# jgdumas/plinopt

Measured on AMD Instinct MI355X. Metric: candidate SLPs/sec, higher is better.
Workload: dtype u32

## Files before the change

plinopt_amd/csrc/plo_capi.hip:

```cpp
#include "plo_cse_wave.hip"
#include "plo_cse_batch.hip"
#include "plo_kmethod.hip"
#include "plo_kmethod_batch.hip"
#include "plo_cse_big.hip"
#include "plo_cob.hip"
#include "plo_tril.hip"
#include "plo_lin.hip"
#include "plo_orbit.hip"
#include "plo_orbit_cse.hip"
#include "plo_orbit_growth.hip"
#include "plo_dep.hip"
#include "plo_brent.hip"
#include "../../include/plinopt_hip.h"

#include <algorithm>
#include <atomic>
#include <thread>
#include <chrono>
#include <cstdio>
#include <cstring>
#include <dlfcn.h>
#include <functional>
#include <array>
#include <map>
// ... 560 lines not shown
        for (size_t k = 0; k < rv.size(); ++k) iv[k] = (uint16_t)(std::lower_bound(rv.begin(), rv.end(), inv_mod(rv[k], p)) - rv.begin());
        if ((rc = upload(pl, rv, &B.rval)) || (rc = upload(pl, rt, &B.rtid)) || (rc = upload(pl, iv, &B.invid))) return rc;
        B.nr = (uint32_t)rv.size(); B.mode = 2u;
    }
    B.invtab = nullptr;
    if (p <= (1u << 20)) {
        std::vector<uint32_t> it(p, 0); it[1] = 1;
        for (uint32_t i = 2; i < p; ++i) it[i] = (uint32_t)((uint64_t)(p - p / i) * it[p % i] % p);
        if ((rc = upload(pl, it, &B.invtab))) return rc;
    }
    layout_big_workspace(B, K.wide.has_value());
    if ((rc = size_big_lds(pl, K))) return rc;
    HIPCHK(hipFuncSetAttribute(big_kernel_fn(B), hipFuncAttributeMaxDynamicSharedMemorySize, (int)pl->big_lds));
    if (!pl->d_err) HIPCHK(hipMalloc((void **)&pl->d_err, sizeof(uint32_t)));
    if (!pl->d_best) HIPCHK(hipMalloc((void **)&pl->d_best, sizeof(unsigned long long)));
    if (!pl->d_next) HIPCHK(hipMalloc((void **)&pl->d_next, sizeof(unsigned long long)));
    if (!pl->d_stats) HIPCHK(hipMalloc((void **)&pl->d_stats, plo::BS_COUNT * sizeof(uint32_t)));
    B.selcap = PLO_BIG_SELCAP;
    if (K.selcap) B.selcap = (uint32_t)std::min<long>(PLO_BIG_SELCAP, std::max<long>(1, *K.selcap));
    pl->big = true; pl->waves_per_wg = PLO_BIG_THREADS / 64; pl->lds_bytes = pl->big_lds + (uint32_t)sizeof(plo::BigShared);
    return PLO_OK;
}

int rebuild_big_plan(plo_plan *pl)
{
    for (void *d : pl->big_bufs) (void)hipFree(d);
    pl->big_bufs.clear();
    if (pl->d_ws) { (void)hipFree(pl->d_ws); pl->d_ws = nullptr; pl->ws_slices = 0; }
    return build_big_plan(pl);
}

void print_big_stats(const plo_plan *pl)
{
    using namespace plo;
    uint32_t hs[BS_COUNT] = {0};
    if (hipMemcpy(hs, pl->d_stats, sizeof hs, hipMemcpyDeviceToHost) != hipSuccess) return;
    const uint32_t ncand = hs[BS_SUM_CANDIDATES], *mg = hs + BS_LAST_MERGE_US, *ms = hs + BS_LAST_MERGE_SUM_US, *ph = hs + BS_LAST_PHASE_US, *pg = hs + BS_LAST_PGEN_PHASE_US;
    if (pl->B.defer && ncand) fprintf(stderr, "# big kernel, deferred updates: per candidate %.1f merges (%.2f forced by log/hot pressure), %.0f log records, %.0f hot-table updates; last candidate, merge us: hot->log %u, partition pass %u, sum + write back %u, window %u\n",
            (double)hs[BS_SUM_FULLSCANS] / ncand, (double)hs[BS_SUM_FORCED_MERGES] / ncand, ((double)hs[BS_SUM_LOG_HI] * 4294967296.0 + hs[BS_SUM_LOG_LO]) / ncand, (double)hs[BS_SUM_HOTOPS] / ncand, mg[0], mg[1], mg[2], mg[3]);
    if (pl->B.defer && hs[BS_LAST_MERGE_GROUPS]) fprintf(stderr, "#   merge, sum + write back of the last candidate: %u groups; us: sum (loads + table) %u, scan + write back %u, clear + bounds %u\n", hs[BS_LAST_MERGE_GROUPS], ms[0], ms[1], ms[3]);
    fprintf(stderr, "# big kernel (last candidate): steps %u, full scans %u, level rebuilds %u; phase us: level %u select %u rows %u sweep1 %u flush1 %u sweep2 %u flush2 %u tail %u\n",
            hs[BS_LAST_STEPS], hs[BS_LAST_FULLSCANS], hs[BS_LAST_REBUILDS], ph[0], ph[1], ph[2], ph[3], ph[4], ph[5], ph[6], ph[7]);
    fprintf(stderr, "# big kernel (last candidate): image load + CSE phase %u us, ProgramGen %u us\n", hs[BS_LAST_CSE_US], hs[BS_LAST_PGEN_US]);
    fprintf(stderr, "# big kernel (last candidate): image load alone %u us; ProgramGen us: table fill + flags %u, expand + A1 %u, A2 %u, A3 + B + count %u, Triangle set-up %u, Triangle %u, D %u\n",
            hs[BS_LAST_LOAD_US], pg[0], pg[1], pg[2], pg[3], pg[4], pg[5], pg[6]);
#ifdef PLO_BIG_PROFILE
    { unsigned long long g2[40] = {0}; if (hipMemcpyFromSymbol(g2, HIP_SYMBOL(plo::g_prof2), sizeof g2) == hipSuccess && g2[32]) {
        static const char *cls[4] = {">=256", "64..255", "16..63", "<16"};
        for (int c_ = 0; c_ < 4; ++c_) { fprintf(stderr, "#   rows/step %-8s ms per candidate: level %.1f select %.1f rows %.1f sweep %.1f flush1 %.1f flush2 %.1f tail %.1f\n", cls[c_],
            g2[c_ * 8 + 0] / 1e5 / g2[32], g2[c_ * 8 + 1] / 1e5 / g2[32], g2[c_ * 8 + 2] / 1e5 / g2[32], g2[c_ * 8 + 3] / 1e5 / g2[32], g2[c_ * 8 + 4] / 1e5 / g2[32], (g2[c_ * 8 + 6] + g2[c_ * 8 + 5]) / 1e5 / g2[32], g2[c_ * 8 + 7] / 1e5 / g2[32]); } } }
    { unsigned long long gp[16] = {0};
      if (hipMemcpyFromSymbol(gp, HIP_SYMBOL(plo::g_prof), sizeof gp) != hipSuccess) memset(gp, 0, sizeof gp);
      if (gp[3]) fprintf(stderr, "#   sweep of the steps with >= 256 rows, all candidates: %llu trips by %llu wave-sweeps; cycles per trip: chunk wait + stores %.0f, aggregation of both chunks %.0f, rest of the loop %.0f; per wave-sweep %.0f cycles, %.1f trips; probe rounds per trip %.2f, active lanes per trip %.1f\n", gp[3], gp[5], (double)gp[0] / gp[3], (double)gp[1] / gp[3], (double)gp[2] / gp[3], (double)gp[4] / gp[5], (double)gp[3] / gp[5], (double)gp[6] / gp[3], (double)gp[7] / gp[3]);
      if (gp[3] && pl->B.defer && pl->B.mode == 2u) fprintf(stderr, "#   aggregation of a trip (lane 0 of every wave, big steps), cycles: ratio-id lookup %.0f, pair read %.0f, compare-and-swap %.0f, bitmap + count %.0f\n", (double)gp[14] / gp[3], (double)gp[8] / gp[3], (double)gp[9] / gp[3], (double)gp[10] / gp[3]);
      if ((gp[14] || gp[15]) && !pl->B.defer) fprintf(stderr, "#   flush 1, all candidates: entries whose pair with a has a as SECOND column %llu, with b %llu\n", gp[14], gp[15]);
      if (gp[11]) fprintf(stderr, "#   flush 1 of the steps with >= 256 rows: %llu wave-trips by %llu wave-flushes; cycles per trip: fetch + decode %.0f, probe loads %.0f, stores + bookkeeping %.0f; per wave-flush %.0f cycles, %.1f trips\n", gp[11], gp[13], (double)gp[8] / gp[11], (double)gp[9] / gp[11], (double)gp[10] / gp[11], (double)gp[12] / gp[13], (double)gp[11] / gp[13]);
    }
    { const uint32_t *s1 = hs + BS_PROF_SWEEP1_US, *s2 = hs + BS_PROF_SWEEP2_US, *nb = hs + BS_PROF_STEPS;
      fprintf(stderr, "#   steps by rows/step [>=256, 64.., 16.., <16]: %u %u %u %u; sweep1 us %u %u %u %u; sweep2 us %u %u %u %u; fallbacks %u %u; flushed keys %u %u\n",
            nb[0], nb[1], nb[2], nb[3], s1[0], s1[1], s1[2], s1[3], s2[0], s2[1], s2[2], s2[3], hs[BS_PROF_FALLBACK1], hs[BS_PROF_FALLBACK2], hs[BS_PROF_FLUSHED1], hs[BS_PROF_FLUSHED2]); }
#endif
}

int launch_big(plo_plan *pl, plo::BigJob J, plo_stats_t *st)
{
    const BigLaunchKnobs K;
    uint64_t per_cu = 2;
    if (K.wg_per_cu) per_cu = std::max<uint64_t>(1, (uint64_t)*K.wg_per_cu);
    uint64_t want = std::min<uint64_t>(J.ncand, (uint64_t)g_cus * per_cu);
    if (K.slices) want = std::min<uint64_t>(want, (uint64_t)*K.slices);
    if (want == 0) want = 1;
    if (pl->ws_slices < want) {
        if (pl->d_ws) { (void)hipFree(pl->d_ws); pl->d_ws = nullptr; pl->ws_slices = 0; }
        size_t fr = 0, tot = 0; HIPCHK(hipMemGetInfo(&fr, &tot));
        uint64_t fit = (uint64_t)(fr * 0.85) / pl->B.ws_stride;
        if (fit == 0) return fail(PLO_E_CAPACITY, "not enough HBM for one candidate workspace");
        want = std::min(want, fit);
        HIPCHK(hipMalloc(&pl->d_ws, want * pl->B.ws_stride));
        pl->ws_slices = want;
    }
    const uint64_t grid = std::min<uint64_t>(pl->ws_slices, want);
    pl->B.ws = (uint8_t *)pl->d_ws;
    HIPCHK(hipMemsetAsync(pl->d_next, 0, sizeof(unsigned long long), g_stream));
    HIPCHK(hipMemsetAsync(pl->d_stats, 0, plo::BS_COUNT * sizeof(uint32_t), g_stream));
    J.err = pl->d_err; J.next = pl->d_next; J.stats = pl->d_stats;
    void *args[] = {&pl->B, &J};
    const int err = checked_launch(pl->d_err, st, LaunchShape{grid, pl->lds_bytes, pl->waves_per_wg, pl->algo_bytes},
                                   [&] { (void)hipLaunchKernel(big_kernel_fn(pl->B), dim3((uint32_t)grid), dim3(PLO_BIG_THREADS), args, pl->big_lds, g_stream); });
    if (err < 0) return err;
    if (K.stats) print_big_stats(pl);
    if (err == plo::BERR_TABLE && !pl->B.defer && pl->big_cap_scale < 256u) {
        pl->big_cap_scale *= 4u; ++pl->big_refits;
        const int rc = rebuild_big_plan(pl);
        return rc != PLO_OK ? rc : launch_big(pl, J, st);
    }
    if (err == plo::BERR_TABLE && pl->B.defer && !pl->big_no_defer) {
        pl->big_no_defer = true; ++pl->big_refits;
        const int rc = rebuild_big_plan(pl);
        return rc != PLO_OK ? rc : launch_big(pl, J, st);
    }
    if (err) {
        static const char *names[] = {"pair table", "frequency/row-count mismatch", "column bound", "level list", "window list", "multiplier list", "tie selection", "ProgramGen"};
        uint32_t site = 0; (void)hipMemcpy(&site, pl->d_stats + plo::BS_ERR_SITE, sizeof site, hipMemcpyDeviceToHost);
        return fail(err == plo::BERR_COLS || err == plo::BERR_DM || err == plo::BERR_HL ? PLO_E_CAPACITY : err == plo::BERR_PGEN ? PLO_E_UNSUPPORTED : PLO_E_INTERNAL,
                    std::string("device (HBM variant): ") + (err >= 11 && err <= 18 ? names[err - 11] : "unknown") + " error " + std::to_string(err) + (site ? " (site " + std::to_string(site) + ")" : ""));
    }
    return PLO_OK;
// ... 2456 lines not shown
```

plinopt_amd/csrc/plo_cse_big.hip:

```cpp
#include <hip/hip_runtime.h>
#include <stdint.h>
#include <type_traits>

namespace plo {

#ifndef PLO_BIG_THREADS
#define PLO_BIG_THREADS 512
#endif
#define PLO_BIG_SELCAP 512u
#define PLO_GVB 16u
#define PLO_GVMASK 0xFFFFull
#define PLO_GEMPTY 0xFFFFFFFFFFFF0000ull

struct BigPlan {
    uint32_t m, n, nnz, p, NCmax, hbits, rb, bb, unit, maxf0, M0, multcap, dmcap, hlcap, scr_stride, aggbits, mers, agg_cb, agg_dual, selcap, prune;
    uint64_t mu;
    uint32_t nv, vt_lds;
    uint32_t mode, nr;
    const uint16_t *rtid, *invid;
    const uint32_t *rval;
    const uint32_t *rs, *ent0, *tptr, *trows, *ucount0, *hist0;
    const uint2 *vt;
    const uint32_t *invtab;
    const uint64_t *tab0;
// ... 272 lines not shown
            continue;
        }
        s = (s + 2u) & mask; pr += 2u;
    }
    const unsigned long long cm = __builtin_amdgcn_ballot_w64(claimed != 0xFFFFFFFFu);
    if (cm) {
        const uint32_t lane = threadIdx.x & 63u, leader = (uint32_t)__builtin_ctzll(cm);
        uint32_t base = 0;
        if (lane == leader) base = wg_add(aggn, (uint32_t)__builtin_popcountll(cm));
        base = (uint32_t)__builtin_amdgcn_readlane((int)base, (int)leader);
        if (claimed != 0xFFFFFFFFu) {
            const uint32_t idx = base + (uint32_t)__builtin_popcountll(cm & ((1ull << lane) - 1ull));
            if (idx < listcap) agglist[idx] = (uint16_t)claimed;
        }
    }
    return done;
}

#define PLO_RIDB 10u
#define PLO_RSTRIDE 32u
struct BigTabs { const uint2 *vts; const uint16_t *rtid; const uint32_t *rval; const uint16_t *invid; uint16_t *list; uint32_t *bloom; };
__device__ __forceinline__ bool agg_add_rid(uint32_t *aggk, uint32_t *aggc32, uint32_t aggbits, uint32_t key, uint32_t *aggn, uint16_t *agglist, uint32_t listcap) {
    const uint32_t mask = (1u << aggbits) - 1u;
    uint32_t s = (key * 0x9E3779B1u) >> (32u - aggbits);
    uint32_t claimed = 0xFFFFFFFFu; bool done = false;
    for (uint32_t pr = 0; pr < PLO_AGG_PROBES;) {
        const uint32_t s1 = (s + 1u) & mask;
        const uint32_t k0 = __hip_atomic_load(&aggk[s], __ATOMIC_RELAXED, __HIP_MEMORY_SCOPE_WORKGROUP), k1 = __hip_atomic_load(&aggk[s1], __ATOMIC_RELAXED, __HIP_MEMORY_SCOPE_WORKGROUP);
        const bool hit0 = k0 == key, emp0 = k0 == 0xFFFFFFFFu, first = hit0 || emp0;
        const bool hit = hit0 || (!emp0 && k1 == key), emp = emp0 || (!hit && k1 == 0xFFFFFFFFu);
        const uint32_t t = first ? s : s1;
        if (hit) { wg_add(&aggc32[t >> 1], 1u << ((t & 1u) << 4)); done = true; break; }
        if (emp) {
            const uint32_t old = wg_cas(&aggk[t], 0xFFFFFFFFu, key);
            if (old == 0xFFFFFFFFu || old == key) { if (old != key) claimed = t; wg_add(&aggc32[t >> 1], 1u << ((t & 1u) << 4)); done = true; break; }
            continue;
        }
        s = (s + 2u) & mask; pr += 2u;
    }
    const unsigned long long cm = __builtin_amdgcn_ballot_w64(claimed != 0xFFFFFFFFu);
    if (cm) {
        const uint32_t lane = threadIdx.x & 63u, leader = (uint32_t)__builtin_ctzll(cm);
        uint32_t base = 0;
        if (lane == leader) base = wg_add(aggn, (uint32_t)__builtin_popcountll(cm));
        base = (uint32_t)__builtin_amdgcn_readlane((int)base, (int)leader);
        if (claimed != 0xFFFFFFFFu) {
            const uint32_t idx = base + (uint32_t)__builtin_popcountll(cm & ((1ull << lane) - 1ull));
            if (idx < listcap) agglist[idx] = (uint16_t)claimed;
        }
    }
    return done;
}

__device__ __forceinline__ bool agg_add_rid_bm(uint32_t *aggk, uint32_t *aggc32, uint32_t aggbits, uint32_t key, uint32_t *bm, uint32_t hshift, uint32_t *iters = nullptr) {
    const uint32_t pmask = (1u << (aggbits - 1u)) - 1u;
    uint32_t pi = (uint32_t)__umul24(key, 0x9E3779u) >> hshift;
    for (uint32_t left = PLO_AGG_PROBES / 2u;;) {
        if (iters) ++*iters;
        const unsigned long long kk = __hip_atomic_load((unsigned long long *)aggk + pi, __ATOMIC_RELAXED, __HIP_MEMORY_SCOPE_WORKGROUP);
        const uint32_t k0 = (uint32_t)kk, k1 = (uint32_t)(kk >> 32);
        const bool first = k0 == key || k0 == 0xFFFFFFFFu;
        const uint32_t kt = first ? k0 : k1;
        bool mine = kt == key;
        const uint32_t next = !mine && kt != 0xFFFFFFFFu ? 1u : 0u;
        if (kt == 0xFFFFFFFFu) {
            const uint32_t sec = first ? 0u : 1u;
            const uint32_t old = wg_cas((uint32_t *)((unsigned long long *)aggk + pi) + sec, 0xFFFFFFFFu, key);
            if (old == 0xFFFFFFFFu) { const uint32_t t = 2u * pi + sec; wg_or(&bm[t >> 5], 1u << (t & 31u)); }
            mine = old == 0xFFFFFFFFu || old == key;
        }
        if (mine) wg_add(&aggc32[pi], first ? 1u : 0x10000u);
        pi = (pi + next) & pmask; left -= next;
        if (mine || left == 0u) return mine;
    }
}

#ifdef PLO_BIG_PROFILE
__device__ __forceinline__ bool agg_add_rid_first_prof(uint32_t *aggk, uint32_t *aggc32, uint32_t aggbits, uint32_t key, uint32_t *bm, unsigned long long *acc) {
    const unsigned long long c0 = clock64();
    const uint32_t s = ((uint32_t)__umul24(key, 0x9E3779u) >> (32u - aggbits)) & ~1u;
    const unsigned long long kk = __hip_atomic_load((unsigned long long *)(aggk + s), __ATOMIC_RELAXED, __HIP_MEMORY_SCOPE_WORKGROUP);
    const uint32_t k0 = (uint32_t)kk, k1 = (uint32_t)(kk >> 32);
    asm volatile("s_waitcnt lgkmcnt(0)" ::: "memory"); const unsigned long long c1 = clock64();
    const bool hit0 = k0 == key, hit = hit0 || k1 == key, emp0 = k0 == 0xFFFFFFFFu, tryc = !hit && (emp0 || k1 == 0xFFFFFFFFu);
    const uint32_t sec = hit ? (hit0 ? 0u : 1u) : (emp0 ? 0u : 1u), t = s + sec;
    uint32_t old = 0u;
    if (tryc) old = wg_cas(&aggk[t], 0xFFFFFFFFu, key);
    asm volatile("s_waitcnt lgkmcnt(0)" ::: "memory"); const unsigned long long c2 = clock64();
    const bool fresh = tryc && old == 0xFFFFFFFFu, ok = hit || fresh || (tryc && old == key);
    if (fresh) wg_or(&bm[t >> 5], 1u << (t & 31u));
    if (ok) wg_add(&aggc32[s >> 1], sec ? 0x10000u : 1u);
    asm volatile("s_waitcnt lgkmcnt(0)" ::: "memory"); const unsigned long long c3 = clock64();
    acc[0] += c1 - c0; acc[1] += c2 - c1; acc[2] += c3 - c2;
    return !ok;
}
#endif

#define PLO_ECOL(e_) ((e_) & 0x7FFFu)
#define PLO_EUNIT(e_) (((e_) >> 15) & 1u)
#define PLO_EVI(e_) ((e_) >> 16)
#define PLO_RW_LEN 0x3FFFu
#define PLO_RW_NEW 0x1F8000u
#define PLO_RW_VIB 22u
#define PLO_RW_VIA 27u
template <class ENT> __device__ __forceinline__ int row_find(ENT ent, uint32_t base, uint32_t L, uint32_t c) {
    uint32_t lo = 0, hi = L;
    while (lo < hi) { uint32_t mid = (lo + hi) >> 1; if (PLO_ECOL(ent[base + mid]) < c) lo = mid + 1; else hi = mid; }
    return (lo < L && PLO_ECOL(ent[base + lo]) == c) ? (int)lo : -1;
}

struct BigShared {
    uint32_t M, theta, ncols, nbadd, nbmul, nmult, naff, dmcount, hlcount, rng, errflag, sel_n, sel_over, invr, fullscans, rebuilds, steps, hlbad, acc0, acc1;
    uint32_t a, b, r, aggn, nspill, keepn; uint64_t kprime; uint64_t selkey;
    uint32_t nbisect, spilltot, listover, nwin, nsearched;
    uint32_t logn, hotn, hotbits, nforced, hotops, logtot_lo, logtot_hi;
    uint32_t derr; unsigned long long tmg[4], tmb[4]; uint32_t ngrp, nloop; uint32_t outcnt[64];
    uint32_t cblk[512];
    unsigned long long tph[8];
    unsigned long long tpg[7], tld;
#ifdef PLO_BIG_PROFILE
    unsigned long long tb1[4], tb2[4]; uint32_t nb[4], fb1, fb2, fl1, fl2;
    unsigned long long tpc[4][8];
    unsigned long long pw[16];
#endif
    uint32_t part[8];
    uint64_t sel[PLO_BIG_SELCAP];
};

#define BSYNC() __syncthreads()
#ifdef PLO_BIG_PROFILE
#define PLO_STAMP(q_) do { if (threadIdx.x == 0) { unsigned long long t_ = wall_clock64(); sh.tph[q_] += t_ - tstamp; sh.tpc[sh.M >= 256u ? 0 : sh.M >= 64u ? 1 : sh.M >= 16u ? 2 : 3][q_] += t_ - tstamp; tstamp = t_; } } while (0)
#else
#define PLO_STAMP(q_) do { if (threadIdx.x == 0) { unsigned long long t_ = wall_clock64(); sh.tph[q_] += t_ - tstamp; tstamp = t_; } } while (0)
#endif

#define PLO_DLB 13u
#define PLO_DCH 4096u
#define PLO_DBIAS 0x8000u
#define PLO_DBLOOM_WORDS 4096u
#define PLO_DMREG_WORDS 16384u
#define PLO_DPMAX 2048u
#define PLO_LEMPTY (~0ull)
static_assert(PLO_DPMAX <= 4u * PLO_BIG_THREADS && PLO_DCH % PLO_BIG_THREADS == 0u && 2u * PLO_DCH + 3u * PLO_DPMAX <= PLO_DMREG_WORDS, "merge layout");
// ... 236 lines not shown
        sh.M = Mx >= 2u ? Mx : 0u; sh.theta = th; sh.hotbits = hb; sh.hotn = 0u; sh.hlcount = 0u; sh.logn = 0u; sh.hlbad = 0u; ++sh.fullscans;
    }
    BSYNC();
    if (sh.errflag) return;
    {
        const uint32_t hb = sh.hotbits, th = sh.theta;
        for (uint32_t s = tid; s < (1u << hb); s += nth) hot[s] = PLO_GEMPTY;
        for (uint32_t w = tid; w < PLO_DBLOOM_WORDS; w += nth) mreg[w] = 0u;
        PLO_BIG_FENCE(); BSYNC();
        if (sh.M >= 2u) {
            for (uint32_t q = wave; q < Pn; q += nwaves) {
                const uint32_t n = pcount[q];
                uint64_t *sp = store + (uint64_t)q * rcap;
                for (uint32_t e0 = 0; e0 < n; e0 += 256u) {
                    uint64_t v[4];
#pragma unroll
                    for (uint32_t u = 0; u < 4u; ++u) { const uint32_t e = e0 + u * 64u + lane; v[u] = e < n ? sp[e] : 0ull; }
#pragma unroll
                    for (uint32_t u = 0; u < 4u; ++u) {
                        const uint32_t e = e0 + u * 64u + lane, c = (uint32_t)(v[u] & 0x7FFFull);
                        if (e < n && c >= th) {
                            const uint64_t k = v[u] >> 16;
                            if (hot_addn(hot, k, c, hb, &sh.hotn) != 0u) { wg_max(&sh.errflag, (uint32_t)BERR_TABLE); wg_max(&sh.derr, 106u); }
                            dbloom_set(mreg, k);
                            const uint32_t idx = wg_add(&sh.hlcount, 1u);
                            if (idx < hlcap) HL[idx] = k; else wg_max(&sh.errflag, (uint32_t)BERR_HL);
                            sp[e] = v[u] & ~0x7FFFull;
                        }
                    }
                }
            }
        }
    }
    PLO_BIG_FENCE(); BSYNC();
    PLO_MSTAMP(3);
#undef PLO_MSTAMP
}

template <int MODE, bool DEFER, bool IDK, class O> __device__ __forceinline__ uint64_t big_candidate(const BigPlan &P, uint8_t *ws, uint64_t seed, BigShared &sh, uint32_t *hist, uint64_t *agg, uint32_t aggbits, const BigTabs &TB, uint32_t *errw)
{
    const uint32_t tid = threadIdx.x, nth = blockDim.x, lane = tid & 63u, wave = tid >> 6, nwaves = nth >> 6;
    typedef WsArr<uint32_t, O> A32; typedef WsArr<uint64_t, O> A64;
    auto tab = [&] { if constexpr (DEFER) return A64{ws, ws_off<O>(P.o_hot)}; else return (uint64_t *)(ws + P.o_tab); }();
    const A64 dlog{ws, ws_off<O>(P.o_log)}; uint32_t *bloom = TB.bloom;
    const A32 ent{ws, ws_off<O>(P.o_ent)};
    const A32 len{ws, ws_off<O>(P.o_len)}, ucount{ws, ws_off<O>(P.o_ucount)}, cntM{ws, ws_off<O>(P.o_cntM)};
    const A64 DM{ws, ws_off<O>(P.o_dm)}, HL{ws, ws_off<O>(P.o_hl)};
    const uint2 *vtg = PW(vt); const uint2 *vts = TB.vts;
    auto VT = [&](uint32_t vi) -> uint2 { if constexpr (MODE == 1) return vts[vi]; else return vtg[vi]; };
    const uint16_t *rtid = TB.rtid, *invid = TB.invid; const uint32_t *rval = TB.rval;
    uint32_t *aggk = (uint32_t *)agg, *aggc32 = aggk + (1u << aggbits); uint16_t *aggc16 = (uint16_t *)aggc32;
    const A32 aff{ws, ws_off<O>(P.o_aff)}, ncrptr{ws, ws_off<O>(P.o_ncrptr)}, ncr{ws, ws_off<O>(P.o_ncr)};
    constexpr bool FAST = MODE == 2 && DEFER;
    uint32_t *aggbm = (uint32_t *)sh.sel;
    uint16_t *agglist = (MODE == 2 && !DEFER) ? TB.list : (uint16_t *)sh.sel; const uint32_t listcap = (MODE == 2 && !DEFER) ? (1u << aggbits) : PLO_AGG_LIST;
    const A64 spill{ws, ws_off<O>(P.o_spill)}; const uint32_t spillcap = PW(nnz) + 64u;
    const A32 multc{ws, ws_off<O>(P.o_multc)}, multv{ws, ws_off<O>(P.o_multv)};
    const uint32_t p = PW(p), rb = PW(rb), kb = IDK ? PW(kb) : rb, abits = kb + PW(bb), n = PW(n), m = PW(m), mers = PW(mers);
    uint32_t hbits = DEFER ? PW(hotbits_min) : PW(hbits);
    const uint64_t mu = PW(mu), cap = 1ull << PW(hbits);
    const uint32_t nr_ = (MODE == 2 && IDK) ? PW(nr) : 0u;
    auto key_ratio = [&](uint32_t x) -> uint32_t {
        if constexpr (MODE == 2 && IDK) { uint32_t lo = 0, hi = nr_; while (lo < hi) { const uint32_t mid = (lo + hi) >> 1; if (rval[mid] < x) lo = mid + 1u; else hi = mid; } return lo; }
        else return x;
    };
#define BKEY(a_, b_, r_) (((uint64_t)(a_) << abits) | ((uint64_t)(b_) << kb) | (uint64_t)key_ratio(r_))

    const unsigned long long tld0 = wall_clock64();
    {
        const uint4 *s4 = (const uint4 *)PW(tab0); uint4 *d4 = (uint4 *)tab;
        const uint64_t n4 = DEFER ? 0ull : cap >> 1;
        for (uint64_t s = tid; s < n4; s += 4ull * nth) {
            uint4 x0 = s4[s], x1, x2, x3; const bool b1 = s + nth < n4, b2 = s + 2ull * nth < n4, b3 = s + 3ull * nth < n4;
            if (b1) x1 = s4[s + nth]; if (b2) x2 = s4[s + 2ull * nth]; if (b3) x3 = s4[s + 3ull * nth];
            d4[s] = x0; if (b1) d4[s + nth] = x1; if (b2) d4[s + 2ull * nth] = x2; if (b3) d4[s + 3ull * nth] = x3;
        }
        const uint32_t q4 = (PW(nnz) + 3u) >> 2;
        const uint4 *e4 = (const uint4 *)PW(ent0); uint4 *de = (uint4 *)ent;
        for (uint32_t k = tid; k < q4; k += 2u * nth) { uint4 x = e4[k], y; const bool b1 = k + nth < q4; if (b1) y = e4[k + nth]; de[k] = x; if (b1) de[k + nth] = y; }
    }
    if constexpr (DEFER) {
        const A32 pcount{ws, ws_off<O>(P.o_pcount)}, ptail{ws, ws_off<O>(P.o_ptail)};
        const uint32_t Pn = 1u << PW(pbits), capp = PW(capp), rcap = capp + PW(plcap); const uint32_t *const pcount0 = PW(pcount0); const uint64_t *const st0 = PW(st0);
        for (uint32_t q = tid; q < Pn; q += nth) { pcount[q] = pcount0[q]; ptail[q] = pcount0[q]; }
        uint64_t *store = (uint64_t *)(ws + P.o_store);
        for (uint32_t q = wave; q < Pn; q += nwaves) {
            const uint32_t nq = pcount0[q]; const uint64_t *sp = st0 + (uint64_t)q * capp; uint64_t *dp = store + (uint64_t)q * rcap;
            for (uint32_t e = lane; e < nq; e += 128u) { const uint64_t x0 = sp[e], x1 = e + 64u < nq ? sp[e + 64u] : 0ull; dp[e] = x0; if (e + 64u < nq) dp[e + 64u] = x1; }
        }
    }
    const A32 tl{ws, ws_off<O>(P.o_tl)}, clen{ws, ws_off<O>(P.o_clen)}, keep{ws, ws_off<O>(P.o_keep)};
    {
        const uint32_t q4 = (PW(nnz) + 3u) >> 2;
        const uint4 *t4 = (const uint4 *)PW(trows); uint4 *d4 = (uint4 *)tl;
        for (uint32_t k = tid; k < q4; k += 2u * nth) { uint4 x = t4[k], y; const bool b1 = k + nth < q4; if (b1) y = t4[k + nth]; d4[k] = x; if (b1) d4[k + nth] = y; }
    }
    {
        const uint32_t *const rs = PW(rs), *const ucount0 = PW(ucount0), *const tptr = PW(tptr), *const hist0 = PW(hist0); const uint32_t NCmax = PW(NCmax), maxf0 = PW(maxf0);
        for (uint32_t i = tid; i < m; i += nth) len[i] = rs[i + 1] - rs[i];
        for (uint32_t c = tid; c < NCmax; c += nth) { ucount[c] = c < n ? ucount0[c] : 0u; cntM[c] = 0u; clen[c] = c < n ? tptr[c + 1] - tptr[c] : 0u; }
        for (uint32_t f = tid; f <= maxf0; f += nth) hist[f] = hist0[f];
    }
    const uint32_t acb = PW(agg_cb); const uint64_t AEMPTY = ~0ull << acb;
    if constexpr (MODE == 2) { for (uint32_t s = tid; s < (1u << aggbits); s += nth) { aggk[s] = 0xFFFFFFFFu; aggc16[s] = 0; } }
    else for (uint32_t s = tid; s < (1u << aggbits); s += nth) agg[s] = AEMPTY;
    if (tid == 0) {
        uint64_t x = seed + 0x9E3779B97F4A7C15ull;
// ... 140 lines not shown
            }
            BSYNC();
            if (sh.errflag) break;
            const uint32_t a = sh.a;
            const uint32_t dn = sh.dmcount < dmcap ? sh.dmcount : dmcap;
            for (uint32_t k = tid; k < dn; k += nth) {
                const uint64_t key = DM[k];
                if ((uint32_t)(key >> abits) == a && gtab_find(tab, key, hbits) == M) {
                    uint32_t idx = wg_add(&sh.sel_n, 1u);
                    if (idx < selcap) sh.sel[idx] = key; else sh.sel_over = 1u;
                }
            }
            BSYNC();
            if (sh.sel_over) {
                if (tid == 0) ++sh.nbisect;
                uint64_t lo = (uint64_t)a << abits, hi = (((uint64_t)a + 1ull) << abits) - 1ull;
                while (lo < hi) {
                    const uint64_t mid = lo + ((hi - lo) >> 1);
                    if (tid == 0) sh.sel_n = 0;
                    BSYNC();
                    uint32_t c = 0;
                    for (uint32_t k = tid; k < dn; k += nth) {
                        const uint64_t key = DM[k];
                        if ((uint32_t)(key >> abits) == a && key <= mid && gtab_find(tab, key, hbits) == M) ++c;
                    }
                    if (c) wg_add(&sh.sel_n, c);
                    BSYNC();
                    const uint32_t tot = sh.sel_n;
                    BSYNC();
                    if ((uint64_t)tot >= sh.kprime + 1ull) hi = mid; else lo = mid + 1ull;
                }
                if (tid == 0) sh.selkey = lo;
            } else {
                const uint32_t sn = sh.sel_n;
                for (uint32_t x = tid; x < sn; x += nth) {
                    const uint64_t mine = sh.sel[x]; uint32_t rank = 0;
                    for (uint32_t y = 0; y < sn; ++y) rank += (sh.sel[y] < mine) ? 1u : 0u;
                    if ((uint64_t)rank == sh.kprime) sh.selkey = mine;
                }
                if (tid == 0 && (uint64_t)sn <= sh.kprime) wg_max(&sh.errflag, (uint32_t)BERR_SEL);
            }
            BSYNC();
            if (sh.errflag) break;
        }
        const uint64_t key = sh.selkey;
        PLO_STAMP(1);
        const uint32_t rfield = (uint32_t)(key & ((1ull << kb) - 1ull)), b = (uint32_t)(key >> kb) & ((1u << bb) - 1u), a = (uint32_t)(key >> abits);
        uint32_t r = rfield; if constexpr (MODE == 2 && IDK) r = rval[rfield];
        const uint32_t lm = ncols;
        if (lm + 1u >= NCmax) { if (tid == 0) wg_max(&sh.errflag, (uint32_t)BERR_COLS); BSYNC(); break; }
        const bool swap = gload32(&ucount[a]) < gload32(&ucount[b]);
        const uint32_t l0 = swap ? b : a, l1 = swap ? a : b;
        if (tid == 0) { sh.naff = 0; sh.aggn = 0; sh.nspill = 0; sh.keepn = 0; }
        if constexpr (FAST) { for (uint32_t w = tid; w < ((1u << aggbits) + 31u) / 32u; w += nth) aggbm[w] = 0u; }
        BSYNC();
#define RL(v_, k_) ((uint32_t)__builtin_amdgcn_readlane((int)(v_), (int)(k_)))
        {
            const A32 la = a < n ? tl + tptr[a] : ncr + ncrptr[a - n], lb = b < n ? tl + tptr[b] : ncr + ncrptr[b - n];
            const uint32_t na = gload32(&clen[a]), nb = gload32(&clen[b]);
            const bool walk_a = na <= nb;
            const A32 lst = walk_a ? la : lb; const uint32_t ln = walk_a ? na : nb;
            if (tid == 0) sh.nsearched += ln;
            const A32 newrows = ncr + ncrptr[lm - n];
            auto emit = [&](uint32_t i, uint32_t base, uint32_t L, uint32_t pa, uint32_t pb, uint32_t ea, uint32_t eb) -> bool {
                uint32_t inv_r;
                if constexpr (MODE == 2) {
                    if (rval[rtid[PLO_EVI(eb) * PLO_RSTRIDE + PLO_EVI(ea)]] != r) return false;
                    inv_r = rval[rtid[PLO_EVI(ea) * PLO_RSTRIDE + PLO_EVI(eb)]];
                } else {
                    const uint2 A = VT(PLO_EVI(ea)), B = VT(PLO_EVI(eb));
                    if (B.x != bmul(r, A.x, p, mu, mers)) return false;
                    inv_r = bmul(A.x, B.y, p, mu, mers);
                }
                const uint32_t idx = wg_add(&sh.naff, 1u);
#ifdef PLO_BIG_PROFILE
                atomicAdd(&sh.tb2[1], 100ull * L);
#endif
                if constexpr (MODE == 2) {
                    *(uint4 *)(aff + 4u * idx) = make_uint4(pa | (pb << 16), base, L | ((swap ? eb : ea) & PLO_RW_NEW) | (PLO_EVI(eb) << PLO_RW_VIB) | (PLO_EVI(ea) << PLO_RW_VIA), i);
                } else {
                uint32_t *rec = &aff[8u * idx];
                *(uint4 *)rec = make_uint4(i, pa | (pb << 16), base, L);
                *(uint2 *)(rec + 4) = make_uint2(ea, eb);
                }
                newrows[idx] = i;
                if (idx == 0) sh.invr = inv_r;
                len[i] = L - 1u;
                if (PLO_EUNIT(ea)) wg_sub(&ucount[a], 1u);
                if (PLO_EUNIT(eb)) wg_sub(&ucount[b], 1u);
                if (PLO_EUNIT(swap ? eb : ea)) wg_add(&ucount[lm], 1u);
                return true;
            };
            auto keep_row = [&](uint32_t i, bool has_col, bool affected) { if (has_col && !affected) keep[wg_add(&sh.keepn, 1u)] = i; };
#ifdef PLO_BIG_PROFILE
            if (tid == 0) { sh.tb2[0] += 100ull * ln; sh.tb2[2] += 100ull * (na <= nb ? nb : na); }
#endif
            for (uint32_t k = tid; k < ln; k += 2u * nth) {
                const bool two = k + nth < ln;
                const uint32_t i0 = lst[k], i1 = two ? lst[k + nth] : i0;
                const uint32_t bs0 = rs[i0], bs1 = rs[i1], L0 = len[i0], L1 = two ? len[i1] : 0u;
                uint32_t lo[4] = {0u, 0u, 0u, 0u}, hi[4] = {L0, L0, L1, L1}, ev[4] = {0xFFFFFFFFu, 0xFFFFFFFFu, 0xFFFFFFFFu, 0xFFFFFFFFu};
                for (;;) {
                    uint32_t v[4], mid[4]; bool any = false;
#pragma unroll
                    for (int q = 0; q < 4; ++q) {
                        mid[q] = (lo[q] + hi[q]) >> 1; const bool go = lo[q] < hi[q]; any |= go;
                        v[q] = go ? ent[(q < 2 ? bs0 : bs1) + mid[q]] : 0u;
                    }
                    if (!any) break;
#pragma unroll
                    for (int q = 0; q < 4; ++q)
                        if (lo[q] < hi[q]) { if (PLO_ECOL(v[q]) < ((q & 1) ? b : a)) lo[q] = mid[q] + 1u; else { hi[q] = mid[q]; ev[q] = v[q]; } }
                }
                {   const bool fa = PLO_ECOL(ev[0]) == a && lo[0] < L0, fb = PLO_ECOL(ev[1]) == b && lo[1] < L0;
                    const bool aff0 = fa && fb && emit(i0, bs0, L0, lo[0], lo[1], ev[0], ev[1]);
                    keep_row(i0, walk_a ? fa : fb, aff0); }
                if (two) { const bool fa = PLO_ECOL(ev[2]) == a && lo[2] < L1, fb = PLO_ECOL(ev[3]) == b && lo[3] < L1;
                    const bool aff1 = fa && fb && emit(i1, bs1, L1, lo[2], lo[3], ev[2], ev[3]);
                    keep_row(i1, walk_a ? fa : fb, aff1); }
            }
        }
        PLO_BIG_FENCE(); BSYNC();
        const uint32_t naff = sh.naff;
        {
            const uint32_t nk = sh.keepn, lc = gload32(&clen[a]) <= gload32(&clen[b]) ? a : b;
            const A32 dst = lc < n ? tl + tptr[lc] : ncr + ncrptr[lc - n];
            for (uint32_t k = tid; k < nk; k += nth) dst[k] = keep[k];
            BSYNC();
            if (tid == 0) clen[lc] = nk;
        }
        PLO_STAMP(2);
        if (naff != M) { if (tid == 0) wg_max(&sh.errflag, (uint32_t)BERR_FREQ); BSYNC(); break; }
        {
#ifdef PLO_BIG_PROFILE
            uint32_t probe_iters = 0; unsigned long long pq[3] = {0, 0, 0}, prt = 0;
#endif
            uint32_t aggsh = 33u - aggbits; asm("" : "+v"(aggsh));
            const uint32_t agg_dual = MODE == 2 ? 0u : PW(agg_dual), logcap = DEFER ? PW(logcap) : 0u;
            auto retire_entry = [&](uint32_t e, uint32_t rw, bool above, uint2 VA, uint2 VB, bool noagg = false) {
                const uint32_t c = PLO_ECOL(e);
                uint32_t x, y, q2, ins;
                if constexpr (MODE == 2) {
                    const uint32_t vi = PLO_EVI(e), via = rw >> PLO_RW_VIA;
#ifdef PLO_BIG_PROFILE
                    const unsigned long long cr0 = clock64();
#endif
                    const uint32_t xid = rtid[((above ? vi : via) * PLO_RSTRIDE) | (above ? via : vi)];
#ifdef PLO_BIG_PROFILE
                    if constexpr (FAST) {
                        asm volatile("s_waitcnt lgkmcnt(0)" ::: "memory"); prt += clock64() - cr0;
                        const bool pend = agg_add_rid_first_prof(aggk, aggc32, aggbits, (c << PLO_RIDB) | xid, aggbm, pq);
                        if (!__builtin_amdgcn_ballot_w64(pend)) return;
                        if (!pend || agg_add_rid_bm(aggk, aggc32, aggbits, (c << PLO_RIDB) | xid, aggbm, aggsh, &probe_iters)) return;
                    }
#else
                    if constexpr (FAST) { if (!noagg) { if (__builtin_expect(agg_add_rid_bm(aggk, aggc32, aggbits, (c << PLO_RIDB) | xid, aggbm, aggsh), 1)) return; } }
#endif
                    else if (agg_add_rid(aggk, aggc32, aggbits, (c << PLO_RIDB) | xid, &sh.aggn, agglist, listcap)) return;
                    const uint32_t vib = (rw >> PLO_RW_VIB) & 31u;
                    const uint32_t bc = rval[rtid[vib * PLO_RSTRIDE + vi]];
                    x = rval[xid]; y = rval[rtid[via * PLO_RSTRIDE + vi]];
                    q2 = c < b ? bc : rval[rtid[vi * PLO_RSTRIDE + vib]];
                    ins = l0 == a ? y : bc;
                } else {
                    const uint2 V = VT(PLO_EVI(e));
                    y = bmul(VA.x, V.y, p, mu, mers);
                    x = c < a ? y : bmul(V.x, VA.y, p, mu, mers);
                    const uint64_t cx = ((uint64_t)c << rb) | x;
                    if (agg_add(agg, aggbits, acb, agg_dual ? (cx << rb) | y : cx, (uint32_t)cx ^ ((uint32_t)(cx >> 32) * 0x85EBCA6Bu), &sh.aggn, agglist, listcap)) return;
                    q2 = c < b ? bmul(VB.x, V.y, p, mu, mers) : bmul(V.x, VB.y, p, mu, mers);
                    ins = bmul(l0 == a ? VA.x : VB.x, V.y, p, mu, mers);
                }
#ifdef PLO_BIG_PROFILE
                wg_add(&sh.fb1, 1u);
#endif
                const uint64_t k1 = c < a ? BKEY(c, a, x) : BKEY(a, c, x);
                const uint64_t k2 = c < b ? BKEY(c, b, q2) : BKEY(b, c, q2);
                if constexpr (DEFER) {
                    for (int w_ = 0; w_ < 2; ++w_) {
                        const uint64_t kk = w_ ? k2 : k1; const uint32_t fc = w_ ? (c < b ? c : b) : (c < a ? c : a);
                        bool done = false;
                        if (dbloom_test(bloom, kk)) {
                            uint64_t v; const uint32_t sl = hot_slot(tab, kk, hbits, v);
                            if (sl != 0xFFFFFFFFu) {
                                const uint32_t o = (uint32_t)(wg_add((unsigned long long *)&tab[sl], ~0ull) & PLO_GVMASK);
                                if (o) { wg_sub(&hist[o], 1u); if (o > 1u) wg_add(&hist[o - 1u], 1u); if (o == M) { wg_sub(&cntM[fc], 1u); wg_sub(&sh.cblk[fc >> 6], 1u); } }
                                else wg_max(&sh.errflag, (uint32_t)BERR_TABLE);
                                done = true;
                            }
                        }
                        if (!done) { const uint32_t li = wg_add(&sh.logn, 1u); if (li < logcap) dlog[li] = PLO_DREC(kk, 1u, false); else wg_max(&sh.errflag, (uint32_t)BERR_TABLE); }
                    }
                    const uint32_t idx = wg_add(&sh.nspill, 1u);
                    if (idx < spillcap) spill[idx] = BKEY(c, lm, ins); else wg_max(&sh.errflag, (uint32_t)BERR_TABLE);
                    return;
                }
                const uint32_t o1 = gtab_dec(tab, k1, hbits);
                if (o1) {
                    wg_sub(&hist[o1], 1u); if (o1 > 1u) wg_add(&hist[o1 - 1u], 1u);
                    if (o1 == M) { wg_sub(&cntM[c < a ? c : a], 1u); wg_sub(&sh.cblk[(c < a ? c : a) >> 6], 1u); }
                }
                const uint32_t o2 = gtab_dec(tab, k2, hbits);
                if (o2) {
                    wg_sub(&hist[o2], 1u); if (o2 > 1u) wg_add(&hist[o2 - 1u], 1u);
                    if (o2 == M) { wg_sub(&cntM[c < b ? c : b], 1u); wg_sub(&sh.cblk[(c < b ? c : b) >> 6], 1u); }
                }
                const uint32_t idx = wg_add(&sh.nspill, 1u);
                if (idx < spillcap) spill[idx] = BKEY(c, lm, ins); else wg_max(&sh.errflag, (uint32_t)BERR_TABLE);
            };
// ... 128 lines not shown
                        { const unsigned long long t2_ = clock64(); pw0 += t1_ - t0_; pw1 += t2_ - t1_; pw2 += t0_ - tl_; tl_ = t2_; ++ptr; }
#endif
                        if (morez) { eA = neA; eB = neB; }
                    }
                    if (lane == 0) {
                        if (LA) ent[baseA + LA - 2u] = (MODE == 2 ? eaA & PLO_RW_NEW : ((l0 == a) ? eaA : ebA) & 0xFFFF8000u) | lm;
                        if (LB) ent[baseB + LB - 2u] = (MODE == 2 ? eaB & PLO_RW_NEW : ((l0 == a) ? eaB : ebB) & 0xFFFF8000u) | lm;
                    }
                    baseA = nbaseA; LA = nLA; baseB = nbaseB; LB = nLB; eA = nfA; eB = nfB;
                }
            }
#ifdef PLO_BIG_PROFILE
            if (lane == 0 && M >= 256u) { atomicAdd(&sh.pw[0], pw0); atomicAdd(&sh.pw[1], pw1); atomicAdd(&sh.pw[2], pw2); atomicAdd(&sh.pw[3], ptr); atomicAdd(&sh.pw[4], clock64() - ts_); atomicAdd(&sh.pw[5], 1ull); atomicAdd(&sh.pw[6], pit); atomicAdd(&sh.pw[7], pact); atomicAdd(&sh.pw[8], pq[0]); atomicAdd(&sh.pw[9], pq[1]); atomicAdd(&sh.pw[10], pq[2]); atomicAdd(&sh.pw[14], prt); }
#endif
        }
#undef RL
        BSYNC();
#ifdef PLO_BIG_PROFILE
        if (tid == 0) { const int cl = M >= 256u ? 0 : M >= 64u ? 1 : M >= 16u ? 2 : 3; sh.tb1[cl] += wall_clock64() - tstamp; ++sh.nb[cl]; }
#endif
        PLO_STAMP(3);
        if constexpr (DEFER) {
            const uint32_t invr = sh.invr, theta = sh.theta;
            const uint32_t maxf0 = PW(maxf0), hlcap = PW(hlcap), dmcap = PW(dmcap), logcap = PW(logcap);
            const uint32_t agg_dual = MODE == 2 ? 0u : PW(agg_dual); const uint32_t *const invtab = MODE == 2 ? nullptr : PW(invtab);
            auto retired = [&](uint64_t k, uint32_t d, uint32_t o) {
                if (o < d) { { wg_max(&sh.errflag, (uint32_t)BERR_TABLE); wg_max(&sh.derr, 201u); } return; }
                wg_sub(&hist[o], 1u); if (o > d) wg_add(&hist[o - d], 1u);
                if (o == M) { wg_sub(&cntM[(uint32_t)(k >> abits)], 1u); wg_sub(&sh.cblk[(uint32_t)(k >> abits) >> 6], 1u); }
            };
            auto inserted = [&](uint64_t k, uint32_t o, uint32_t d) {
                const uint32_t nc = o + d;
                if (nc > maxf0 || nc > M) { wg_max(&sh.errflag, (uint32_t)BERR_FREQ); return; }
                if (o > 0u) wg_sub(&hist[o], 1u);
                wg_add(&hist[nc], 1u);
                if (o < theta && nc >= theta) { uint32_t idx = wg_add(&sh.hlcount, 1u); if (idx < hlcap) HL[idx] = k; else sh.hlbad = 1u; }
                if (nc == M) {
                    wg_add(&cntM[(uint32_t)(k >> abits)], 1u); wg_add(&sh.cblk[(uint32_t)(k >> abits) >> 6], 1u);
                    uint32_t idx = wg_add(&sh.dmcount, 1u);
                    if (idx < dmcap) DM[idx] = k; else wg_max(&sh.errflag, (uint32_t)BERR_DM);
                }
            };
            if (tid == 0) {
                uint64_t v; const uint32_t sl = hot_slot(tab, key, hbits, v);
                if (sl == 0xFFFFFFFFu || (uint32_t)(v & PLO_GVMASK) != M) { wg_max(&sh.errflag, (uint32_t)BERR_TABLE); wg_max(&sh.derr, 202u); }
                else { gstore64(&tab[sl], v - (uint64_t)M); retired(key, M, M); }
            }
            const uint32_t nent = sh.aggn, nslot = FAST ? (1u << aggbits) / 16u : nent <= listcap ? nent : (1u << aggbits);
            uint32_t nhot = 0;
            for (uint32_t s0 = 0; s0 < nslot; s0 += nth) {
              const uint32_t e_ = s0 + tid;
              uint32_t bits_ = 0;
              if constexpr (FAST) {
                  if (e_ < nslot) bits_ = (aggbm[e_ >> 1] >> ((e_ & 1u) << 4)) & 0xFFFFu;
              }
              for (bool more_ = true; more_;) {
                bool valid; uint32_t s;
                if constexpr (FAST) { valid = bits_ != 0u; s = valid ? e_ * 16u + (uint32_t)__builtin_ctz(bits_) : 0u; bits_ &= bits_ - 1u; }
                else { valid = e_ < nslot; s = valid ? (nent <= listcap ? (uint32_t)agglist[e_] : e_) : 0u; }
                uint32_t c = 0, x = 0, y = 0, d = 0;
                if constexpr (MODE == 2) {
                    const uint32_t kq = valid ? aggk[s] : 0xFFFFFFFFu;
                    valid = kq != 0xFFFFFFFFu;
                    if (valid) {
                        d = aggc16[s]; aggk[s] = 0xFFFFFFFFu; aggc16[s] = 0; c = kq >> PLO_RIDB;
                        const uint32_t xid = kq & ((1u << PLO_RIDB) - 1u);
                        x = rval[xid]; y = rval[c > a ? (uint32_t)invid[xid] : xid];
                    }
                } else {
                    const uint64_t v = valid ? agg[s] : AEMPTY;
                    valid = v != AEMPTY;
                    if (valid) {
                        agg[s] = AEMPTY;
                        uint64_t k = v >> acb; d = (uint32_t)(v & ((1ull << acb) - 1ull));
                        if (agg_dual) { y = (uint32_t)(k & ((1ull << rb) - 1ull)); k >>= rb; }
                        c = (uint32_t)(k >> rb); x = (uint32_t)(k & ((1ull << rb) - 1ull));
                        if (!agg_dual) y = c > a ? (invtab ? invtab[x] : binv(x, p, mu, mers)) : x;
                    }
                }
                uint64_t k1 = 0, k2 = 0, k3 = 0;
                if (valid) {
                    const uint32_t ry = bmul(r, y, p, mu, mers);
                    const uint32_t x2 = c < b ? ry : bmul(x, invr, p, mu, mers);
                    k1 = c < a ? BKEY(c, a, x) : BKEY(a, c, x); k2 = c < b ? BKEY(c, b, x2) : BKEY(b, c, x2);
                    k3 = BKEY(c, lm, l0 == a ? y : ry);
                }
                bool c1 = valid, c2 = valid;
                if (valid && dbloom_test(bloom, k1)) {
                    uint64_t v; const uint32_t sl = hot_slot(tab, k1, hbits, v);
                    if (sl != 0xFFFFFFFFu) { const uint32_t o = (uint32_t)(v & PLO_GVMASK); if (o >= d) gstore64(&tab[sl], v - (uint64_t)d); retired(k1, d, o); c1 = false; ++nhot; }
                }
                if (valid && dbloom_test(bloom, k2)) {
                    uint64_t v; const uint32_t sl = hot_slot(tab, k2, hbits, v);
                    if (sl != 0xFFFFFFFFu) { const uint32_t o = (uint32_t)(v & PLO_GVMASK); if (o >= d) gstore64(&tab[sl], v - (uint64_t)d); retired(k2, d, o); c2 = false; ++nhot; }
                }
                const bool h3 = valid && d >= theta, c3 = valid && !h3 && d >= 2u;
                if (h3) {
                    const uint32_t o = hot_addn(tab, k3, d, hbits, &sh.hotn);
                    if (o != 0u) { wg_max(&sh.errflag, (uint32_t)BERR_TABLE); wg_max(&sh.derr, 203u); } else { inserted(k3, 0u, d); dbloom_set(bloom, k3); ++nhot; }
                }
                dlog_append3(dlog, &sh.logn, logcap, c1, PLO_DREC(k1, d, false), c2, PLO_DREC(k2, d, false), c3, PLO_DREC(k3, d, true), &sh.errflag);
                if constexpr (FAST) more_ = __builtin_amdgcn_ballot_w64(bits_ != 0u) != 0ull; else more_ = false;
              }
            }
            BSYNC();
            const uint32_t nsp = sh.nspill < spillcap ? sh.nspill : spillcap;
            for (uint32_t e = tid; e < nsp; e += nth) {
                const uint64_t k = spill[e];
                const uint32_t o = hot_addn(tab, k, 1u, hbits, &sh.hotn);
                if (o == 0xFFFFFFFFu) { { wg_max(&sh.errflag, (uint32_t)BERR_TABLE); wg_max(&sh.derr, 204u); } continue; }
                inserted(k, o, 1u); dbloom_set(bloom, k); ++nhot;
// ... 614 lines not shown
```

Before: 1017.

## Drop LDS occupancy bitmap; scan aggregation keys directly and reuse walked list pointer

Removes the per-step occupancy bitmap that was cleared each step and updated with an atomic OR on every fresh insert into the aggregation table. The flush now finds occupied slots by reading the key pairs directly, eight pairs per thread, in a strided layout. The keep-list write-back also reuses the list pointer chosen during the walk instead of reloading clen, and drops one barrier. The trade is fewer LDS atomics and no bitmap clear, in exchange for a full scan of the key array at flush time.

```diff
diff --git a/plinopt_amd/csrc/plo_capi.hip b/plinopt_amd/csrc/plo_capi.hip
--- a/plinopt_amd/csrc/plo_capi.hip
+++ b/plinopt_amd/csrc/plo_capi.hip
@@ -636,7 +636,7 @@
     { unsigned long long gp[16] = {0};
       if (hipMemcpyFromSymbol(gp, HIP_SYMBOL(plo::g_prof), sizeof gp) != hipSuccess) memset(gp, 0, sizeof gp);
       if (gp[3]) fprintf(stderr, "#   sweep of the steps with >= 256 rows, all candidates: %llu trips by %llu wave-sweeps; cycles per trip: chunk wait + stores %.0f, aggregation of both chunks %.0f, rest of the loop %.0f; per wave-sweep %.0f cycles, %.1f trips; probe rounds per trip %.2f, active lanes per trip %.1f\n", gp[3], gp[5], (double)gp[0] / gp[3], (double)gp[1] / gp[3], (double)gp[2] / gp[3], (double)gp[4] / gp[5], (double)gp[3] / gp[5], (double)gp[6] / gp[3], (double)gp[7] / gp[3]);
-      if (gp[3] && pl->B.defer && pl->B.mode == 2u) fprintf(stderr, "#   aggregation of a trip (lane 0 of every wave, big steps), cycles: ratio-id lookup %.0f, pair read %.0f, compare-and-swap %.0f, bitmap + count %.0f\n", (double)gp[14] / gp[3], (double)gp[8] / gp[3], (double)gp[9] / gp[3], (double)gp[10] / gp[3]);
+      if (gp[3] && pl->B.defer && pl->B.mode == 2u) fprintf(stderr, "#   aggregation of a trip (lane 0 of every wave, big steps), cycles: ratio-id lookup %.0f, pair read %.0f, compare-and-swap %.0f, count %.0f\n", (double)gp[14] / gp[3], (double)gp[8] / gp[3], (double)gp[9] / gp[3], (double)gp[10] / gp[3]);
       if ((gp[14] || gp[15]) && !pl->B.defer) fprintf(stderr, "#   flush 1, all candidates: entries whose pair with a has a as SECOND column %llu, with b %llu\n", gp[14], gp[15]);
       if (gp[11]) fprintf(stderr, "#   flush 1 of the steps with >= 256 rows: %llu wave-trips by %llu wave-flushes; cycles per trip: fetch + decode %.0f, probe loads %.0f, stores + bookkeeping %.0f; per wave-flush %.0f cycles, %.1f trips\n", gp[11], gp[13], (double)gp[8] / gp[11], (double)gp[9] / gp[11], (double)gp[10] / gp[11], (double)gp[12] / gp[13], (double)gp[11] / gp[13]);
     }
diff --git a/plinopt_amd/csrc/plo_cse_big.hip b/plinopt_amd/csrc/plo_cse_big.hip
--- a/plinopt_amd/csrc/plo_cse_big.hip
+++ b/plinopt_amd/csrc/plo_cse_big.hip
@@ -348,7 +348,7 @@
     return done;
 }
 
-__device__ __forceinline__ bool agg_add_rid_bm(uint32_t *aggk, uint32_t *aggc32, uint32_t aggbits, uint32_t key, uint32_t *bm, uint32_t hshift, uint32_t *iters = nullptr) {
+__device__ __forceinline__ bool agg_add_rid_bm(uint32_t *aggk, uint32_t *aggc32, uint32_t aggbits, uint32_t key, uint32_t hshift, uint32_t *iters = nullptr) {
     const uint32_t pmask = (1u << (aggbits - 1u)) - 1u;
     uint32_t pi = (uint32_t)__umul24(key, 0x9E3779u) >> hshift;
     for (uint32_t left = PLO_AGG_PROBES / 2u;;) {
@@ -362,7 +362,6 @@
         if (kt == 0xFFFFFFFFu) {
             const uint32_t sec = first ? 0u : 1u;
             const uint32_t old = wg_cas((uint32_t *)((unsigned long long *)aggk + pi) + sec, 0xFFFFFFFFu, key);
-            if (old == 0xFFFFFFFFu) { const uint32_t t = 2u * pi + sec; wg_or(&bm[t >> 5], 1u << (t & 31u)); }
             mine = old == 0xFFFFFFFFu || old == key;
         }
         if (mine) wg_add(&aggc32[pi], first ? 1u : 0x10000u);
@@ -372,7 +371,7 @@
 }
 
 #ifdef PLO_BIG_PROFILE
-__device__ __forceinline__ bool agg_add_rid_first_prof(uint32_t *aggk, uint32_t *aggc32, uint32_t aggbits, uint32_t key, uint32_t *bm, unsigned long long *acc) {
+__device__ __forceinline__ bool agg_add_rid_first_prof(uint32_t *aggk, uint32_t *aggc32, uint32_t aggbits, uint32_t key, unsigned long long *acc) {
     const unsigned long long c0 = clock64();
     const uint32_t s = ((uint32_t)__umul24(key, 0x9E3779u) >> (32u - aggbits)) & ~1u;
     const unsigned long long kk = __hip_atomic_load((unsigned long long *)(aggk + s), __ATOMIC_RELAXED, __HIP_MEMORY_SCOPE_WORKGROUP);
@@ -383,8 +382,7 @@
     uint32_t old = 0u;
     if (tryc) old = wg_cas(&aggk[t], 0xFFFFFFFFu, key);
     asm volatile("s_waitcnt lgkmcnt(0)" ::: "memory"); const unsigned long long c2 = clock64();
-    const bool fresh = tryc && old == 0xFFFFFFFFu, ok = hit || fresh || (tryc && old == key);
-    if (fresh) wg_or(&bm[t >> 5], 1u << (t & 31u));
+    const bool ok = hit || (tryc && (old == 0xFFFFFFFFu || old == key));
     if (ok) wg_add(&aggc32[s >> 1], sec ? 0x10000u : 1u);
     asm volatile("s_waitcnt lgkmcnt(0)" ::: "memory"); const unsigned long long c3 = clock64();
     acc[0] += c1 - c0; acc[1] += c2 - c1; acc[2] += c3 - c2;
@@ -727,7 +725,6 @@
     uint32_t *aggk = (uint32_t *)agg, *aggc32 = aggk + (1u << aggbits); uint16_t *aggc16 = (uint16_t *)aggc32;
     const A32 aff{ws, ws_off<O>(P.o_aff)}, ncrptr{ws, ws_off<O>(P.o_ncrptr)}, ncr{ws, ws_off<O>(P.o_ncr)};
     constexpr bool FAST = MODE == 2 && DEFER;
-    uint32_t *aggbm = (uint32_t *)sh.sel;
     uint16_t *agglist = (MODE == 2 && !DEFER) ? TB.list : (uint16_t *)sh.sel; const uint32_t listcap = (MODE == 2 && !DEFER) ? (1u << aggbits) : PLO_AGG_LIST;
     const A64 spill{ws, ws_off<O>(P.o_spill)}; const uint32_t spillcap = PW(nnz) + 64u;
     const A32 multc{ws, ws_off<O>(P.o_multc)}, multv{ws, ws_off<O>(P.o_multv)};
@@ -974,14 +971,15 @@
         const bool swap = gload32(&ucount[a]) < gload32(&ucount[b]);
         const uint32_t l0 = swap ? b : a, l1 = swap ? a : b;
         if (tid == 0) { sh.naff = 0; sh.aggn = 0; sh.nspill = 0; sh.keepn = 0; }
-        if constexpr (FAST) { for (uint32_t w = tid; w < ((1u << aggbits) + 31u) / 32u; w += nth) aggbm[w] = 0u; }
         BSYNC();
 #define RL(v_, k_) ((uint32_t)__builtin_amdgcn_readlane((int)(v_), (int)(k_)))
+        A32 wlst; uint32_t lc;
         {
             const A32 la = a < n ? tl + tptr[a] : ncr + ncrptr[a - n], lb = b < n ? tl + tptr[b] : ncr + ncrptr[b - n];
             const uint32_t na = gload32(&clen[a]), nb = gload32(&clen[b]);
             const bool walk_a = na <= nb;
             const A32 lst = walk_a ? la : lb; const uint32_t ln = walk_a ? na : nb;
+            wlst = lst; lc = walk_a ? a : b;
             if (tid == 0) sh.nsearched += ln;
             const A32 newrows = ncr + ncrptr[lm - n];
             auto emit = [&](uint32_t i, uint32_t base, uint32_t L, uint32_t pa, uint32_t pb, uint32_t ea, uint32_t eb) -> bool {
@@ -1045,10 +1043,8 @@
         PLO_BIG_FENCE(); BSYNC();
         const uint32_t naff = sh.naff;
         {
-            const uint32_t nk = sh.keepn, lc = gload32(&clen[a]) <= gload32(&clen[b]) ? a : b;
-            const A32 dst = lc < n ? tl + tptr[lc] : ncr + ncrptr[lc - n];
-            for (uint32_t k = tid; k < nk; k += nth) dst[k] = keep[k];
-            BSYNC();
+            const uint32_t nk = sh.keepn;
+            for (uint32_t k = tid; k < nk; k += nth) wlst[k] = keep[k];
             if (tid == 0) clen[lc] = nk;
         }
         PLO_STAMP(2);
@@ -1071,12 +1067,12 @@
 #ifdef PLO_BIG_PROFILE
                     if constexpr (FAST) {
                         asm volatile("s_waitcnt lgkmcnt(0)" ::: "memory"); prt += clock64() - cr0;
-                        const bool pend = agg_add_rid_first_prof(aggk, aggc32, aggbits, (c << PLO_RIDB) | xid, aggbm, pq);
+                        const bool pend = agg_add_rid_first_prof(aggk, aggc32, aggbits, (c << PLO_RIDB) | xid, pq);
                         if (!__builtin_amdgcn_ballot_w64(pend)) return;
-                        if (!pend || agg_add_rid_bm(aggk, aggc32, aggbits, (c << PLO_RIDB) | xid, aggbm, aggsh, &probe_iters)) return;
+                        if (!pend || agg_add_rid_bm(aggk, aggc32, aggbits, (c << PLO_RIDB) | xid, aggsh, &probe_iters)) return;
                     }
 #else
-                    if constexpr (FAST) { if (!noagg) { if (__builtin_expect(agg_add_rid_bm(aggk, aggc32, aggbits, (c << PLO_RIDB) | xid, aggbm, aggsh), 1)) return; } }
+                    if constexpr (FAST) { if (!noagg) { if (__builtin_expect(agg_add_rid_bm(aggk, aggc32, aggbits, (c << PLO_RIDB) | xid, aggsh), 1)) return; } }
 #endif
                     else if (agg_add_rid(aggk, aggc32, aggbits, (c << PLO_RIDB) | xid, &sh.aggn, agglist, listcap)) return;
                     const uint32_t vib = (rw >> PLO_RW_VIB) & 31u;
@@ -1311,11 +1307,17 @@
               const uint32_t e_ = s0 + tid;
               uint32_t bits_ = 0;
               if constexpr (FAST) {
-                  if (e_ < nslot) bits_ = (aggbm[e_ >> 1] >> ((e_ & 1u) << 4)) & 0xFFFFu;
+                  const uint32_t npair = 1u << (aggbits - 1u);
+#pragma unroll
+                  for (uint32_t u = 0; u < 8u; ++u) {
+                      const uint32_t q = s0 * 8u + u * nth + tid; const bool in = q < npair;
+                      const uint2 kq2 = ((const uint2 *)aggk)[in ? q : 0u];
+                      bits_ |= in ? ((kq2.x != 0xFFFFFFFFu ? 1u : 0u) | (kq2.y != 0xFFFFFFFFu ? 2u : 0u)) << (2u * u) : 0u;
+                  }
               }
               for (bool more_ = true; more_;) {
                 bool valid; uint32_t s;
-                if constexpr (FAST) { valid = bits_ != 0u; s = valid ? e_ * 16u + (uint32_t)__builtin_ctz(bits_) : 0u; bits_ &= bits_ - 1u; }
+                if constexpr (FAST) { valid = bits_ != 0u; const uint32_t j_ = valid ? (uint32_t)__builtin_ctz(bits_) : 0u; s = valid ? 2u * (s0 * 8u + (j_ >> 1) * nth + tid) + (j_ & 1u) : 0u; bits_ &= bits_ - 1u; }
                 else { valid = e_ < nslot; s = valid ? (nent <= listcap ? (uint32_t)agglist[e_] : e_) : 0u; }
                 uint32_t c = 0, x = 0, y = 0, d = 0;
                 if constexpr (MODE == 2) {
```

After: 1040, median of 6. 2.3% higher.
